# xiaojino/RUArt

Hardware: AMD Instinct MI355X
Metric: VQA samples/sec fwd+bwd (B=64, q=30, ocr=100) (higher is better)
Workload: dtype f16 MFMA + block-scaled fp8 (e4m3) MFMA correction, f32 accumulate / residual stream

## Files before the change

ruart_amd/csrc/sdnet_gemm.hip:

```cpp
#include <cstdlib>
#include "common.h"
#include "ruart_hip.h"

#define XBK 32
template <int TM> struct XT {
  static constexpr int THREADS = TM * 2;
  static constexpr int WN = TM / 64;
  static constexpr int JT = TM / 32;
  static constexpr int TRS = TM * 2 + 16;
  static constexpr int ARR = 32 * TRS;
};

typedef __attribute__((__vector_size__(4 * sizeof(short)))) short xtr16x4_t;
typedef __attribute__((address_space(3))) xtr16x4_t* xtr_ptr_t;

namespace {

__device__ __forceinline__ void split_bf16(float x, bf16_t& hi, bf16_t& lo) {
  hi = (bf16_t)x;
  lo = (bf16_t)(x - (float)hi);
}

__device__ __forceinline__ int kc_off(int r, int chunk ) {
  const int line = r >> 1;
  return line * 128 + ((((r & 1) * 4 + chunk) ^ (line & 7)) << 4);
}

template <int TM, int MODE, int VW, bool MASKED = false>
struct Stager {
  float v[16];
  unsigned mb[MASKED ? 16 / VW : 1];
  unsigned ok;

  __device__ __forceinline__ static void ldv(const float* p, float* out) {
    if (VW == 4) {
      const f32x4_t t = *reinterpret_cast<const f32x4_t*>(p);
      out[0] = t[0]; out[1] = t[1]; out[2] = t[2]; out[3] = t[3];
    } else if (VW == 2) {
      typedef float f32x2v __attribute__((ext_vector_type(2)));
      const f32x2v t = *reinterpret_cast<const f32x2v*>(p);
      out[0] = t[0]; out[1] = t[1];
    } else {
      out[0] = *p;
    }
  }
  __device__ __forceinline__ static unsigned ldm(const unsigned char* p) {
    if (VW == 4) return *reinterpret_cast<const unsigned*>(p);
    if (VW == 2) return *reinterpret_cast<const unsigned short*>(p);
    return *p;
  }

  __device__ __forceinline__ static int div_rpm(int x, float inv) { return (int)(((float)x + 0.5f) * inv); }

  __device__ __forceinline__ static void mask_rows(int (&mo)[4], int r0, int rows, int K, int tid, int rpm) {
    const float inv = 1.0f / (float)rpm;
#pragma unroll
    for (int p = 0; p < 4; ++p) mo[p] = div_rpm(min(r0 + p * (TM / 4) + (tid >> 3), rows - 1), inv) * K;
  }

  template <bool KFULL>
  __device__ __forceinline__ void load(const float* __restrict__ P, long srow, long sk, int r0, int rows, int k0, int K, int tid,
                                       const unsigned char* __restrict__ S, int rpm, const int (&mo)[4]) {
    ok = KFULL ? 0xffffu : 0u;
    if (MODE == 0) {
      const int kq = (tid & 7) * 4;
      const unsigned pitch = (unsigned)srow;
#pragma unroll
      for (int p = 0; p < 4; ++p) {
        const int r = r0 + p * (TM / 4) + (tid >> 3), k = k0 + kq;
        const unsigned ro = (unsigned)min(r, rows - 1) * pitch;
#pragma unroll
        for (int j = 0; j < 4; j += VW) {
          const int kk = k + j, kc = KFULL ? kk : min(kk, K - VW);
          ldv(P + (ro + (unsigned)kc), &v[p * 4 + j]);
          if (!KFULL && kk < K) ok |= ((1u << VW) - 1u) << (p * 4 + j);
          if (MASKED) mb[(p * 4 + j) / VW] = ldm(S + (unsigned)(mo[p] + kc));
        }
      }
    } else {
      const int m4 = (tid % (TM / 4)) * 4;
      const float inv = 1.0f / (float)rpm;
      const unsigned pitch = (unsigned)sk;
#pragma unroll
      for (int p = 0; p < 4; ++p) {
        const int k = k0 + 2 * (tid / (TM / 4)) + (p & 1) + 16 * (p >> 1), r = r0 + m4;
        const int kc = KFULL ? k : min(k, K - 1);
        const unsigned ko = (unsigned)kc * pitch;
        const unsigned so = MASKED ? (unsigned)(div_rpm(kc, inv) * rows) : 0u;
        if (!KFULL && k < K) ok |= 0xfu << (p * 4);
#pragma unroll
        for (int j = 0; j < 4; j += VW) {
          const int rrc = min(r + j, rows - VW);
          ldv(P + (ko + (unsigned)rrc), &v[p * 4 + j]);
          if (MASKED) mb[(p * 4 + j) / VW] = ldm(S + (so + (unsigned)rrc));
        }
      }
    }
  }

  template <bool KFULL>
  __device__ __forceinline__ void store(char* hi_img, char* lo_img, int tid, bool with_lo = true, float scale = 1.f) const {
#pragma unroll
    for (int p = 0; p < 4; ++p) {
      bf16x4_t h, l;
#pragma unroll
      for (int i = 0; i < 4; ++i) {
        bf16_t a, b;
        const int e = p * 4 + i;
        float x = v[e];
        if (MASKED) x = ((mb[e / VW] >> (8 * (e % VW))) & 0xffu) ? x * scale : 0.f;
        if (!KFULL) x = ((ok >> e) & 1u) ? x : 0.f;
        split_bf16(x, a, b);
        h[i] = a;
        l[i] = b;
      }
      int off;
      if (MODE == 0) {
        const int r = p * (TM / 4) + (tid >> 3), kq = tid & 7;
        off = kc_off(r, kq >> 1) + (kq & 1) * 8;
      } else {
        const int k = 2 * (tid / (TM / 4)) + (p & 1) + 16 * (p >> 1);
        off = k * XT<TM>::TRS + (tid % (TM / 4)) * 8;
      }
      *reinterpret_cast<bf16x4_t*>(hi_img + off) = h;
      if (with_lo) *reinterpret_cast<bf16x4_t*>(lo_img + off) = l;
    }
  }
};

template <int TM, int MODE>
__device__ __forceinline__ bf16x8_t frag(const char* img, int row_base, int fr, int fq) {
  if (MODE == 0) {
    return *reinterpret_cast<const bf16x8_t*>(img + kc_off(row_base + fr, fq));
  } else {
    const char* base = img + (8 * fq + (fr >> 2)) * XT<TM>::TRS + (row_base + (fr & 3) * 4) * 2;
    union { struct { xtr16x4_t a, b; } s; bf16x8_t f; } u;
    u.s.a = __builtin_amdgcn_ds_read_tr16_b64_v4i16((xtr_ptr_t)base);
    u.s.b = __builtin_amdgcn_ds_read_tr16_b64_v4i16((xtr_ptr_t)(base + 4 * XT<TM>::TRS));
    return u.f;
  }
}

template <int TM, int AMODE, int BMODE, int VWA, int VWB, int NP, int MSK = 0>
__device__ __forceinline__ void x3_tile(const float* __restrict__ A, long sam, long sak, const float* __restrict__ B, long sbk, long sbn,
                                        const float* __restrict__ bias, float* __restrict__ C, int ldc, int M, int N, int K, int splitk,
                                        float* __restrict__ ws, const unsigned char* __restrict__ a_scale, const unsigned char* __restrict__ b_scale,
                                        float keep_scale, const float* __restrict__ c_scale, int rpm, const float* __restrict__ R, int ldr,
                                        int act, int id) {
  typedef XT<TM> T;
  constexpr int ARR = T::ARR, JT = T::JT;
  extern __shared__ __attribute__((aligned(1024))) char smem[];
  const int tid = threadIdx.x, lane = tid & 63, wave = tid >> 6;
  const int wm = wave / T::WN, wn = wave % T::WN;
  const int fr = lane & 15, fq = lane >> 4;
  const int ntn = (N + TM - 1) / TM;
  const int tile = id / splitk, slice = id - tile * splitk;
  const int m0 = (tile / ntn) * TM, n0 = (tile % ntn) * TM;
  const int ksteps = (K + XBK - 1) / XBK;
  const int per = (ksteps + splitk - 1) / splitk;
  const int kbeg = slice * per, kend = min(ksteps, kbeg + per);

  f32x4_t acc[4][JT];
#pragma unroll
  for (int i = 0; i < 4; ++i)
#pragma unroll
    for (int j = 0; j < JT; ++j) acc[i][j] = (f32x4_t){0.f, 0.f, 0.f, 0.f};

  const long a_srow = sam, a_sk = sak, b_srow = sbn, b_sk = sbk;
  auto compute = [&](const char* st) {
#pragma unroll
    for (int jh = 0; jh < JT / 4; ++jh) {
      bf16x8_t ah[4], al[4];
#pragma unroll
      for (int j = 0; j < 4; ++j) {
        ah[j] = frag<TM, AMODE>(st, wm * (TM / 2) + (jh * 4 + j) * 16, fr, fq);
        if (NP == 3) al[j] = frag<TM, AMODE>(st + ARR, wm * (TM / 2) + (jh * 4 + j) * 16, fr, fq);
      }
#pragma unroll
      for (int i = 0; i < 4; ++i) {
        const bf16x8_t bh = frag<TM, BMODE>(st + 2 * ARR, wn * 64 + i * 16, fr, fq);
        bf16x8_t bl = bh;
        if (NP == 3) bl = frag<TM, BMODE>(st + 3 * ARR, wn * 64 + i * 16, fr, fq);
#pragma unroll
        for (int j = 0; j < 4; ++j) {
          f32x4_t& c = acc[i][jh * 4 + j];
          if (NP == 3) {
            c = mfma_16x16x32(bl, ah[j], c);
            c = mfma_16x16x32(bh, al[j], c);
          }
          c = mfma_16x16x32(bh, ah[j], c);
        }
      }
    }
  };
  int moa[4] = {0, 0, 0, 0}, mob[4] = {0, 0, 0, 0};
  if (MSK == 1 && AMODE == 0) Stager<TM, AMODE, VWA, true>::mask_rows(moa, m0, M, K, tid, rpm);
  if (MSK == 2 && BMODE == 0) Stager<TM, BMODE, VWB, true>::mask_rows(mob, n0, N, K, tid, rpm);
  if constexpr (TM == 128) {
    Stager<TM, AMODE, VWA, MSK == 1> sa0, sa1;
    Stager<TM, BMODE, VWB, MSK == 2> sb0, sb1;
    sa0.template load<false>(A, a_srow, a_sk, m0, M, kbeg * XBK, K, tid, a_scale, rpm, moa);
    sb0.template load<false>(B, b_srow, b_sk, n0, N, kbeg * XBK, K, tid, b_scale, rpm, mob);
    sa1.template load<false>(A, a_srow, a_sk, m0, M, (kbeg + 1) * XBK, K, tid, a_scale, rpm, moa);
    sb1.template load<false>(B, b_srow, b_sk, n0, N, (kbeg + 1) * XBK, K, tid, b_scale, rpm, mob);
    char* const st0 = smem;
    char* const st1 = smem + 4 * ARR;
    int t = kbeg;
#define X3_PAIR(KF)                                                                                       \
    {                                                                                                     \
      sa0.template store<KF>(st0, st0 + ARR, tid, NP == 3, keep_scale);                                   \
      sb0.template store<KF>(st0 + 2 * ARR, st0 + 3 * ARR, tid, NP == 3, keep_scale);                     \
      __syncthreads();                 \
      __builtin_amdgcn_sched_barrier(0);                                                                  \
      sa0.template load<KF>(A, a_srow, a_sk, m0, M, (t + 2) * XBK, K, tid, a_scale, rpm, moa);            \
      sb0.template load<KF>(B, b_srow, b_sk, n0, N, (t + 2) * XBK, K, tid, b_scale, rpm, mob);            \
      __builtin_amdgcn_sched_barrier(0);                                                                  \
      compute(st0);                                                                                       \
      __builtin_amdgcn_sched_barrier(0);                                                                  \
      sa1.template store<KF>(st1, st1 + ARR, tid, NP == 3, keep_scale);                                   \
      sb1.template store<KF>(st1 + 2 * ARR, st1 + 3 * ARR, tid, NP == 3, keep_scale);                     \
      __syncthreads();                                                                                    \
      __builtin_amdgcn_sched_barrier(0);                                                                  \
      sa1.template load<KF>(A, a_srow, a_sk, m0, M, (t + 3) * XBK, K, tid, a_scale, rpm, moa);            \
      sb1.template load<KF>(B, b_srow, b_sk, n0, N, (t + 3) * XBK, K, tid, b_scale, rpm, mob);            \
      __builtin_amdgcn_sched_barrier(0);                                                                  \
      compute(st1);                                                                                       \
      __builtin_amdgcn_sched_barrier(0);                                                                  \
    }
    const int kfull = K / XBK;
    for (; t + 1 < kend && t + 3 < kfull; t += 2) X3_PAIR(true)
    for (; t + 1 < kend; t += 2) X3_PAIR(false)
#undef X3_PAIR
    if (t < kend) {
      sa0.template store<false>(st0, st0 + ARR, tid, NP == 3, keep_scale);
      sb0.template store<false>(st0 + 2 * ARR, st0 + 3 * ARR, tid, NP == 3, keep_scale);
      __syncthreads();
      compute(st0);
    }
  } else {
    Stager<TM, AMODE, VWA, MSK == 1> sa;
    Stager<TM, BMODE, VWB, MSK == 2> sb;
    if (kbeg < kend) {
      sa.template load<false>(A, a_srow, a_sk, m0, M, kbeg * XBK, K, tid, a_scale, rpm, moa);
      sb.template load<false>(B, b_srow, b_sk, n0, N, kbeg * XBK, K, tid, b_scale, rpm, mob);
    }
    const int kfull = K / XBK;
    int t = kbeg;
    for (; t + 1 < kend && t + 1 < kfull; ++t) {
      char* st = smem + ((t - kbeg) & 1) * (4 * ARR);
      sa.template store<true>(st, st + ARR, tid, NP == 3, keep_scale);
      sb.template store<true>(st + 2 * ARR, st + 3 * ARR, tid, NP == 3, keep_scale);
      __syncthreads();
      sa.template load<true>(A, a_srow, a_sk, m0, M, (t + 1) * XBK, K, tid, a_scale, rpm, moa);
      sb.template load<true>(B, b_srow, b_sk, n0, N, (t + 1) * XBK, K, tid, b_scale, rpm, mob);
      compute(st);
    }
    for (; t < kend; ++t) {
      char* st = smem + ((t - kbeg) & 1) * (4 * ARR);
      sa.template store<false>(st, st + ARR, tid, NP == 3, keep_scale);
      sb.template store<false>(st + 2 * ARR, st + 3 * ARR, tid, NP == 3, keep_scale);
      __syncthreads();
      if (t + 1 < kend) {
        sa.template load<false>(A, a_srow, a_sk, m0, M, (t + 1) * XBK, K, tid, a_scale, rpm, moa);
        sb.template load<false>(B, b_srow, b_sk, n0, N, (t + 1) * XBK, K, tid, b_scale, rpm, mob);
      }
      compute(st);
    }
  }

  if (splitk > 1) {
    float* slab = ws + ((size_t)tile * splitk + slice) * (TM * TM);
#pragma unroll
    for (int i = 0; i < 4; ++i)
#pragma unroll
      for (int j = 0; j < JT; ++j) *reinterpret_cast<f32x4_t*>(slab + ((i * JT + j) * T::THREADS + tid) * 4) = acc[i][j];
    return;
  }
  const uintptr_t bits = reinterpret_cast<uintptr_t>(C) | (R ? reinterpret_cast<uintptr_t>(R) : 0) | (bias ? reinterpret_cast<uintptr_t>(bias) : 0) |
                         (c_scale ? reinterpret_cast<uintptr_t>(c_scale) : 0);
  const bool vec_all = (bits & 15) == 0 && (ldc & 3) == 0 && (!R || (ldr & 3) == 0) && (!c_scale || (N & 3) == 0);
#pragma unroll
  for (int i = 0; i < 4; ++i) {
    const int n = n0 + wn * 64 + i * 16 + fq * 4;
    if (vec_all && n + 3 < N) {
      f32x4_t bv = {0.f, 0.f, 0.f, 0.f};
      if (bias) bv = *reinterpret_cast<const f32x4_t*>(bias + n);
#pragma unroll
      for (int j = 0; j < JT; ++j) {
        const int m = m0 + wm * (TM / 2) + j * 16 + fr;
        if (m >= M) continue;
        f32x4_t v = acc[i][j] + bv;
        if (act == RUART_ACT_GELU) {
#pragma unroll
          for (int r = 0; r < 4; ++r) v[r] = v[r] * 0.5f * (1.0f + erff(v[r] * 0.70710678118654752440f));
        }
        if (c_scale) v *= *reinterpret_cast<const f32x4_t*>(c_scale + (size_t)(m / rpm) * N + n);
        if (R) v += *reinterpret_cast<const f32x4_t*>(R + (size_t)m * ldr + n);
        *reinterpret_cast<f32x4_t*>(C + (size_t)m * ldc + n) = v;
      }
      continue;
    }
    f32x4_t bv = {0.f, 0.f, 0.f, 0.f};
    if (bias) {
#pragma unroll
      for (int r = 0; r < 4; ++r) bv[r] = (n + r < N) ? bias[n + r] : 0.f;
    }
#pragma unroll
    for (int j = 0; j < JT; ++j) {
      const int m = m0 + wm * (TM / 2) + j * 16 + fr;
      if (m >= M || n >= N) continue;
      f32x4_t v = acc[i][j] + bv;
      if (act == RUART_ACT_GELU) {
#pragma unroll
        for (int r = 0; r < 4; ++r) v[r] = v[r] * 0.5f * (1.0f + erff(v[r] * 0.70710678118654752440f));
      }
      if (c_scale) {
        const float* sp = c_scale + (size_t)(m / rpm) * N + n;
#pragma unroll
        for (int r = 0; r < 4; ++r)
          if (n + r < N) v[r] *= sp[r];
      }
      if (R) {
        const float* rp = R + (size_t)m * ldr + n;
#pragma unroll
        for (int r = 0; r < 4; ++r)
          if (n + r < N) v[r] += rp[r];
      }
      float* dst = C + (size_t)m * ldc + n;
#pragma unroll
      for (int r = 0; r < 4; ++r)
        if (n + r < N) dst[r] = v[r];
    }
  }
}

template <int TM, int AMODE, int BMODE, int VWA, int VWB, int NP = 3, int MSK = 0>
__global__ __launch_bounds__(TM * 2, 2) void gemm_x3_kernel(const float* __restrict__ A, long sam, long sak, const float* __restrict__ B,
                                                            long sbk, long sbn, const float* __restrict__ bias, float* __restrict__ C,
                                                            int ldc, int M, int N, int K, int splitk, float* __restrict__ ws,
                                                            const unsigned char* __restrict__ a_scale,
                                                            const unsigned char* __restrict__ b_scale, float keep_scale,
                                                            const float* __restrict__ c_scale, int rpm, const float* __restrict__ R,
                                                            int ldr, int act) {
  x3_tile<TM, AMODE, BMODE, VWA, VWB, NP, MSK>(A, sam, sak, B, sbk, sbn, bias, C, ldc, M, N, K, splitk, ws, a_scale, b_scale, keep_scale, c_scale,
                                               rpm, R, ldr, act, xcd_remap(blockIdx.x, gridDim.x));
}

#define X3G_MAX 44
struct X3GProb {
  const float* A;
  const float* B;
  float* C;
  float* ws;
  int lda, ldb, ldc, M, N, K, splitk, blk0, red0, accum;
};
struct X3GArgs {
  X3GProb p[X3G_MAX];
  int n;
};
template <bool VECA, bool VECB>
__global__ __launch_bounds__(256, 2) void gemm_x3_grouped_tn_kernel(const X3GArgs g) {
  const int id = xcd_remap(blockIdx.x, gridDim.x);
  int q = 0;
  while (q + 1 < g.n && id >= g.p[q + 1].blk0) ++q;
  const X3GProb& P = g.p[q];
  const float* R = (P.accum && P.splitk == 1) ? P.C : nullptr;
  x3_tile<128, 1, 1, VECA ? 4 : 1, VECB ? 4 : 1, 3>(P.A, 1, P.lda, P.B, P.ldb, 1, nullptr, P.C, P.ldc, P.M, P.N, P.K, P.splitk, P.ws, nullptr, nullptr,
                                    1.f, nullptr, 1, R, P.ldc, RUART_ACT_NONE, id - P.blk0);
}

template <int TM>
__device__ __forceinline__ void x3_reduce_body(const float* __restrict__ ws, const float* __restrict__ bias, float* __restrict__ C, int ldc,
                                               int M, int N, int splitk, const float* __restrict__ c_scale, int rpm,
                                               const float* __restrict__ R, int ldr, int act, int blk) {
  typedef XT<TM> T;
  constexpr int JT = T::JT;
  const int tid = threadIdx.x, lane = tid & 63, wave = tid >> 6;
  const int wm = wave / T::WN, wn = wave % T::WN, fr = lane & 15, fq = lane >> 4;
  const int ntn = (N + TM - 1) / TM;
  const int tile = blk / (4 * JT), ij = blk % (4 * JT), i = ij / JT, j = ij % JT;
  const int m = (tile / ntn) * TM + wm * (TM / 2) + j * 16 + fr, n = (tile % ntn) * TM + wn * 64 + i * 16 + fq * 4;
  if (m >= M || n >= N) return;
  const float* p = ws + (size_t)tile * splitk * (TM * TM) + (ij * T::THREADS + tid) * 4;
  f32x4_t s = {0.f, 0.f, 0.f, 0.f};
  int sl = 0;
  for (; sl + 8 <= splitk; sl += 8) {
    f32x4_t a[8];
#pragma unroll
    for (int u = 0; u < 8; ++u) a[u] = *reinterpret_cast<const f32x4_t*>(p + (size_t)(sl + u) * (TM * TM));
#pragma unroll
    for (int u = 0; u < 8; ++u) s += a[u];
  }
  {
    f32x4_t a[8];
#pragma unroll
    for (int u = 0; u < 8; ++u) a[u] = *reinterpret_cast<const f32x4_t*>(p + (size_t)min(sl + u, splitk - 1) * (TM * TM));
#pragma unroll
    for (int u = 0; u < 8; ++u)
      if (sl + u < splitk) s += a[u];
  }
  const uintptr_t bits = reinterpret_cast<uintptr_t>(C) | (R ? reinterpret_cast<uintptr_t>(R) : 0) | (bias ? reinterpret_cast<uintptr_t>(bias) : 0) |
                         (c_scale ? reinterpret_cast<uintptr_t>(c_scale) : 0);
  const bool vec = n + 3 < N && (bits & 15) == 0 && (ldc & 3) == 0 && (!R || (ldr & 3) == 0) && (!c_scale || (N & 3) == 0);
  if (vec) {
    f32x4_t v = s;
    if (bias) v += *reinterpret_cast<const f32x4_t*>(bias + n);
    if (act == RUART_ACT_GELU) {
#pragma unroll
      for (int r = 0; r < 4; ++r) v[r] = v[r] * 0.5f * (1.0f + erff(v[r] * 0.70710678118654752440f));
    }
    if (c_scale) v *= *reinterpret_cast<const f32x4_t*>(c_scale + (size_t)(m / rpm) * N + n);
    if (R) v += *reinterpret_cast<const f32x4_t*>(R + (size_t)m * ldr + n);
    *reinterpret_cast<f32x4_t*>(C + (size_t)m * ldc + n) = v;
    return;
  }
#pragma unroll
  for (int r = 0; r < 4; ++r)
    if (n + r < N) {
      float v = s[r] + (bias ? bias[n + r] : 0.f);
      if (act == RUART_ACT_GELU) v = v * 0.5f * (1.0f + erff(v * 0.70710678118654752440f));
      if (c_scale) v *= c_scale[(size_t)(m / rpm) * N + n + r];
      if (R) v += R[(size_t)m * ldr + n + r];
      C[(size_t)m * ldc + n + r] = v;
    }
}

template <int TM>
__global__ __launch_bounds__(TM * 2) void x3_reduce_kernel(const float* __restrict__ ws, const float* __restrict__ bias,
                                                           float* __restrict__ C, int ldc, int M, int N, int splitk,
                                                           const float* __restrict__ c_scale, int rpm, const float* __restrict__ R,
                                                           int ldr, int act) {
  x3_reduce_body<TM>(ws, bias, C, ldc, M, N, splitk, c_scale, rpm, R, ldr, act, blockIdx.x);
}

__global__ __launch_bounds__(256) void x3_reduce_grouped_kernel(const X3GArgs g) {
  const int id = blockIdx.x;
  int q = 0;
  while (q + 1 < g.n && id >= g.p[q + 1].red0) ++q;
  const X3GProb& P = g.p[q];
  if (P.splitk <= 1) return;
  x3_reduce_body<128>(P.ws, nullptr, P.C, P.ldc, P.M, P.N, P.splitk, nullptr, 1, P.accum ? P.C : nullptr, P.ldc, RUART_ACT_NONE, id - P.red0);
}

struct Plan { int tm, tiles, splitk; };

Plan make_plan(int M, int N, int K, int amode, int bmode) {
  const int ksteps = (K + XBK - 1) / XBK;
  static const int fill = [] { const char* e = getenv("RUART_X3_FILL"); return e ? atoi(e) : 128; }();
  static const int nosplit = [] { const char* e = getenv("RUART_X3_NOSPLIT_TILES"); return e ? atoi(e) : 160; }();
  auto split_for = [&](int tiles) {
    if (tiles >= nosplit || ksteps < 16) return 1;
    int s = (fill + tiles - 1) / tiles;
    if (s > ksteps / 4) s = ksteps / 4;
    if (s > 64) s = 64;
    return s < 1 ? 1 : s;
  };
  const int t256 = ((M + 255) / 256) * ((N + 255) / 256), t128 = ((M + 127) / 128) * ((N + 127) / 128);
  Plan p;
  static const int fill256 = [] { const char* e = getenv("RUART_X3_T256_FILL"); return e ? atoi(e) : 256; }();
  static const int min256 = [] { const char* e = getenv("RUART_X3_T256_MIN"); return e ? atoi(e) : 192; }();
  int s256 = 1;
  if (t256 < 200 && ksteps >= 16) {
    s256 = (fill256 + t256 - 1) / t256;
    if (s256 > ksteps / 8) s256 = ksteps / 8;
    if (s256 < 1) s256 = 1;
  }
  const double waste = (double)t256 * 65536.0 / ((double)M * N);
  if (bmode == 0 && (long long)M * N >= 4096LL * 1024 && t256 * s256 >= min256 && waste < 1.25) {
    (void)amode;
    p.tm = 256; p.tiles = t256; p.splitk = s256;
  } else {
    p.tm = 128; p.tiles = t128; p.splitk = split_for(t128);
  }
  return p;
}

template <int TM, int AM, int BM_, int VA, int VB, int NP = 3, int MSK = 0>
void launch_x3(const float* A, long sam, long sak, const float* B, long sbk, long sbn, const float* bias, float* C, int ldc, int M,
               int N, int K, const Plan& p, float* ws, const unsigned char* a_scale, const unsigned char* b_scale, float keep_scale,
               const float* c_scale, int rpm,
               const float* R, int ldr, int act, hipStream_t s) {
  auto kern = gemm_x3_kernel<TM, AM, BM_, VA, VB, NP, MSK>;
  constexpr int lds = 2 * 4 * XT<TM>::ARR;
  static bool done = (hipFuncSetAttribute((const void*)kern, hipFuncAttributeMaxDynamicSharedMemorySize, lds), true);
  (void)done;
  hipLaunchKernelGGL(kern, dim3(p.tiles * p.splitk), dim3(XT<TM>::THREADS), lds, s, A, sam, sak, B, sbk, sbn, bias, C, ldc, M, N, K,
                     p.splitk, ws, a_scale, b_scale, keep_scale, c_scale, rpm, R, ldr, act);
  if (p.splitk > 1)
    hipLaunchKernelGGL(x3_reduce_kernel<TM>, dim3(p.tiles * 4 * XT<TM>::JT), dim3(XT<TM>::THREADS), 0, s, ws, bias, C, ldc, M, N, p.splitk,
                       c_scale, rpm, R, ldr, act);
}

}

extern "C" int ruart_gemm_x3_plan(int M, int N, int K, int a_k_contiguous, int b_k_contiguous, int* splitk, size_t* ws_bytes) {
  RUART_ENTRY();
  if (M <= 0 || N <= 0 || K <= 0) return (int)hipErrorInvalidValue;
  const Plan p = make_plan(M, N, K, a_k_contiguous ? 0 : 1, b_k_contiguous ? 0 : 1);
  if (splitk) *splitk = p.splitk;
  if (ws_bytes) *ws_bytes = p.splitk > 1 ? (size_t)p.tiles * p.splitk * p.tm * p.tm * sizeof(float) : 0;
  return 0;
}

namespace {
template <int NP>
int gemm_xn(const float* A, long long sam, long long sak, const float* B, long long sbk, long long sbn,
            const float* bias, const float* residual, int ldr, int act, float* C, int ldc, int M, int N, int K,
            float* ws, size_t ws_bytes, const unsigned char* a_scale, const unsigned char* b_scale, float keep_scale,
            const float* c_scale, int rows_per_scale_row, void* stream) {
  if (!A || !B || !C || M <= 0 || N <= 0 || K <= 0 || ldc < N) return (int)hipErrorInvalidValue;
  if ((residual && ldr < N) || (act != RUART_ACT_NONE && act != RUART_ACT_GELU)) return (int)hipErrorInvalidValue;
  const float* R = residual;
  const int rpm = rows_per_scale_row > 0 ? rows_per_scale_row : 1;
  if ((a_scale && sak != 1) || (b_scale && sbn != 1)) return (int)hipErrorInvalidValue;
  const int amode = (sak == 1) ? 0 : (sam == 1 ? 1 : -1);
  const int bmode = (sbk == 1) ? 0 : (sbn == 1 ? 1 : -1);
  if (amode < 0 || bmode < 0) return (int)hipErrorInvalidValue;
  {
    const long long ea = amode == 0 ? (long long)(M - 1) * sam + K : (long long)(K - 1) * sak + M;
    const long long eb = bmode == 0 ? (long long)(N - 1) * sbn + K : (long long)(K - 1) * sbk + N;
    if (ea >= (1LL << 30) || eb >= (1LL << 30) || sam < 0 || sak < 0 || sbk < 0 || sbn < 0) return (int)hipErrorInvalidValue;
  }
  Plan p = make_plan(M, N, K, amode, bmode);
  if (p.splitk > 1 && (!ws || ws_bytes < (size_t)p.tiles * p.splitk * p.tm * p.tm * sizeof(float))) p.splitk = 1;
  auto width = [](const float* base, long pitch, int extent, const unsigned char* mask) {
    const uintptr_t bits = reinterpret_cast<uintptr_t>(base), mbits = mask ? reinterpret_cast<uintptr_t>(mask) : 0;
    if ((bits & 15) == 0 && (mbits & 3) == 0 && (pitch & 3) == 0 && (extent & 3) == 0) return 4;
    if ((bits & 7) == 0 && (mbits & 1) == 0 && (pitch & 1) == 0 && (extent & 1) == 0) return 2;
    return 1;
  };
  const int vwa = width(A, amode == 0 ? sam : sak, amode == 0 ? K : M, a_scale);
  const int vwb = width(B, bmode == 0 ? sbn : sbk, bmode == 0 ? K : N, b_scale);
  if (p.tm == 256 && (vwa == 1 || vwb == 1)) {
    p.tm = 128;
    p.tiles = ((M + 127) / 128) * ((N + 127) / 128);
    p.splitk = 1;
  }
  hipStream_t s = (hipStream_t)stream;
#define X3L(TM, AM, BM_, VA, VB) \
  launch_x3<TM, AM, BM_, VA, VB, NP>(A, sam, sak, B, sbk, sbn, bias, C, ldc, M, N, K, p, ws, a_scale, b_scale, keep_scale, c_scale, rpm, R, ldr, act, s)
#define X3W(TM, AM, BM_)                                         \
  do {                                                           \
    if (vwa == 4 && vwb == 4) X3L(TM, AM, BM_, 4, 4);            \
    else if (vwa == 4 && vwb == 2) X3L(TM, AM, BM_, 4, 2);       \
    else if (vwa == 2 && vwb == 4) X3L(TM, AM, BM_, 2, 4);       \
    else if (vwa == 2 && vwb == 2) X3L(TM, AM, BM_, 2, 2);       \
    else if (TM == 256) return (int)hipErrorInvalidValue;        \
    else X3S(AM, BM_);                                           \
  } while (0)
#define X3S(AM, BM_)                                             \
  do {                                                           \
    if (vwa == 4) X3L(128, AM, BM_, 4, 1);                       \
    else if (vwa == 2) X3L(128, AM, BM_, 2, 1);                  \
    else if (vwb == 4) X3L(128, AM, BM_, 1, 4);                  \
    else if (vwb == 2) X3L(128, AM, BM_, 1, 2);                  \
    else X3L(128, AM, BM_, 1, 1);                                \
  } while (0)
  if (a_scale || b_scale) {
    if (a_scale && b_scale) return (int)hipErrorInvalidValue;
    const int vw = vwa < vwb ? vwa : vwb;
#define X3M(TM, AM, BM_, VW_, MSK_) \
  launch_x3<TM, AM, BM_, VW_, VW_, NP, MSK_>(A, sam, sak, B, sbk, sbn, bias, C, ldc, M, N, K, p, ws, a_scale, b_scale, keep_scale, c_scale, rpm, R, ldr, act, s)
    if (a_scale && amode == 0 && bmode == 0) {
      if (p.tm == 256 && vw >= 2) {
        if (vw == 4) X3M(256, 0, 0, 4, 1); else X3M(256, 0, 0, 2, 1);
      } else {
        if (p.tm == 256) { p.tm = 128; p.tiles = ((M + 127) / 128) * ((N + 127) / 128); p.splitk = 1; }
        if (vw == 4) X3M(128, 0, 0, 4, 1); else if (vw == 2) X3M(128, 0, 0, 2, 1); else X3M(128, 0, 0, 1, 1);
      }
    } else {
      if (p.tm == 256) { p.tm = 128; p.tiles = ((M + 127) / 128) * ((N + 127) / 128); p.splitk = 1; }
      if (b_scale && amode == 1 && bmode == 1) {
        if (vw == 4) X3M(128, 1, 1, 4, 2); else if (vw == 2) X3M(128, 1, 1, 2, 2); else X3M(128, 1, 1, 1, 2);
      } else if (a_scale && amode == 0 && bmode == 1) X3M(128, 0, 1, 1, 1);
      else if (b_scale && amode == 0 && bmode == 1) X3M(128, 0, 1, 1, 2);
      else return (int)hipErrorInvalidValue;
    }
#undef X3M
  } else if (p.tm == 256) {
    if (bmode != 0) return (int)hipErrorInvalidValue;
    if (amode == 0) X3W(256, 0, 0); else X3W(256, 1, 0);
  } else if (amode == 0 && bmode == 0) X3W(128, 0, 0);
  else if (amode == 0 && bmode == 1) X3W(128, 0, 1);
  else if (amode == 1 && bmode == 0) X3W(128, 1, 0);
  else X3W(128, 1, 1);
#undef X3S
#undef X3W
#undef X3L
  RUART_CHECK_LAUNCH();
  return 0;
}
}

extern "C" int ruart_gemm_x3(const float* A, long long sam, long long sak, const float* B, long long sbk, long long sbn,
                             const float* bias, const float* residual, int ldr, int act, float* C, int ldc, int M, int N, int K,
                             float* ws, size_t ws_bytes, const unsigned char* a_keep, const unsigned char* b_keep, float keep_scale,
                             const float* c_scale, int rows_per_scale_row, void* stream) {
  RUART_ENTRY();
  return gemm_xn<3>(A, sam, sak, B, sbk, sbn, bias, residual, ldr, act, C, ldc, M, N, K, ws, ws_bytes, a_keep, b_keep, keep_scale, c_scale,
                    rows_per_scale_row, stream);
}

extern "C" int ruart_gemm_x1(const float* A, long long sam, long long sak, const float* B, long long sbk, long long sbn,
                             const float* bias, const float* residual, int ldr, int act, float* C, int ldc, int M, int N, int K,
                             float* ws, size_t ws_bytes, const unsigned char* a_keep, const unsigned char* b_keep, float keep_scale,
                             const float* c_scale, int rows_per_scale_row, void* stream) {
  RUART_ENTRY();
  return gemm_xn<1>(A, sam, sak, B, sbk, sbn, bias, residual, ldr, act, C, ldc, M, N, K, ws, ws_bytes, a_keep, b_keep, keep_scale, c_scale,
                    rows_per_scale_row, stream);
}

extern "C" int ruart_gemm_bf16_tn(const float* A, long long sak_rows, const float* B, long long sbk_rows, float* C, int ldc, int M, int N,
                                  int K, float* ws, size_t ws_bytes, void* stream) {
  RUART_ENTRY();
  return gemm_xn<1>(A, 1, sak_rows, B, sbk_rows, 1, nullptr, nullptr, 0, RUART_ACT_NONE, C, ldc, M, N, K, ws, ws_bytes, nullptr, nullptr,
                    1.f, nullptr, 1, stream);
}

extern "C" size_t ruart_gemm_x3_tn_grouped_ws(const ruart_x3_tn_problem* probs, int n) {
  size_t total = 0;
  for (int i = 0; i < n; ++i) {
    const Plan p = make_plan(probs[i].M, probs[i].N, probs[i].K, 1, 1);
    if (p.splitk > 1) total += (size_t)p.tiles * p.splitk * 128 * 128 * sizeof(float);
  }
  return total;
}

extern "C" int ruart_gemm_x3_tn_grouped(const ruart_x3_tn_problem* probs, int n, float* ws, size_t ws_bytes, void* stream) {
  RUART_ENTRY();
  if (n <= 0 || !probs) return (int)hipErrorInvalidValue;
  if (ruart_gemm_x3_tn_grouped_ws(probs, n) > ws_bytes) return (int)hipErrorInvalidValue;
  hipStream_t s = (hipStream_t)stream;
  size_t ws_off = 0;
  for (int cls = 0; cls < 4; ++cls) {
    const bool va = cls & 1, vb = cls & 2;
    X3GArgs g;
    g.n = 0;
    int blk = 0, red = 0;
    auto flush = [&]() -> int {
      if (g.n == 0) return 0;
      constexpr int lds = 2 * 4 * XT<128>::ARR;
#define X3G_LAUNCH(VA, VB)                                                                                                  \
  do {                                                                                                                       \
    auto kern = gemm_x3_grouped_tn_kernel<VA, VB>;                                                                           \
    static bool done = (hipFuncSetAttribute((const void*)kern, hipFuncAttributeMaxDynamicSharedMemorySize, lds), true);    \
    (void)done;                                                                                                              \
    hipLaunchKernelGGL(kern, dim3(blk), dim3(256), lds, s, g);                                                               \
  } while (0)
      if (va && vb) X3G_LAUNCH(true, true);
      else if (va) X3G_LAUNCH(true, false);
      else if (vb) X3G_LAUNCH(false, true);
      else X3G_LAUNCH(false, false);
#undef X3G_LAUNCH
      hipError_t e = hipGetLastError();
      if (e != hipSuccess) return (int)e;
      if (red > 0) {
        hipLaunchKernelGGL(x3_reduce_grouped_kernel, dim3(red), dim3(256), 0, s, g);
        e = hipGetLastError();
        if (e != hipSuccess) return (int)e;
      }
      g.n = 0;
      blk = red = 0;
      return 0;
    };
    for (int i = 0; i < n; ++i) {
      const ruart_x3_tn_problem& q = probs[i];
      if (!q.A || !q.B || !q.C || q.M <= 0 || q.N <= 0 || q.K <= 0 || q.lda < q.M || q.ldb < q.N || q.ldc < q.N ||
          (long long)q.K * q.lda >= (1LL << 30) || (long long)q.K * q.ldb >= (1LL << 30))
        return (int)hipErrorInvalidValue;
      const bool qa = ((reinterpret_cast<uintptr_t>(q.A) & 15) == 0) && ((q.lda & 3) == 0) && ((q.M & 3) == 0);
      const bool qb = ((reinterpret_cast<uintptr_t>(q.B) & 15) == 0) && ((q.ldb & 3) == 0) && ((q.N & 3) == 0);
      if (qa != va || qb != vb) continue;
      const Plan pl = make_plan(q.M, q.N, q.K, 1, 1);
      X3GProb& P = g.p[g.n];
      P.A = q.A; P.B = q.B; P.C = q.C;
      P.lda = q.lda; P.ldb = q.ldb; P.ldc = q.ldc;
      P.M = q.M; P.N = q.N; P.K = q.K;
      P.splitk = pl.splitk;
      P.accum = q.accumulate ? 1 : 0;
      P.blk0 = blk;
      P.red0 = red;
      P.ws = nullptr;
      if (pl.splitk > 1) {
        P.ws = ws + ws_off / sizeof(float);
        ws_off += (size_t)pl.tiles * pl.splitk * 128 * 128 * sizeof(float);
        red += pl.tiles * 4 * XT<128>::JT;
      }
      blk += pl.tiles * pl.splitk;
      if (++g.n == X3G_MAX) {
        const int rc = flush();
        if (rc) return rc;
      }
    }
    const int rc = flush();
    if (rc) return rc;
  }
  return 0;
}
```

Measured before the change: 2895.

## Use unaligned 4-wide loads with edge shifting instead of alignment-gated width dispatch

Replaces the alignment-based vector-width selection (4/2/1) in the fp32-input GEMM staging with a single rule: use 4-wide loads whenever the extent is at least 4, using unaligned vector types. Edge tiles clamp the load start and then shift the loaded lanes in registers to realign them, so misaligned or odd-sized operands no longer fall back to scalar or 2-wide loads or drop from 256 to 128 tiles. The epilogue and split-K reduce also drop the alignment check and use unaligned 4-wide stores. This adds select logic at edge tiles and relies on unaligned global accesses being cheap.

```diff
diff --git a/ruart_amd/csrc/sdnet_gemm.hip b/ruart_amd/csrc/sdnet_gemm.hip
--- a/ruart_amd/csrc/sdnet_gemm.hip
+++ b/ruart_amd/csrc/sdnet_gemm.hip
@@ -26,27 +26,29 @@
   return line * 128 + ((((r & 1) * 4 + chunk) ^ (line & 7)) << 4);
 }
 
+typedef float f32x4u_t __attribute__((ext_vector_type(4), aligned(4)));
+
 template <int TM, int MODE, int VW, bool MASKED = false>
 struct Stager {
+  static_assert(VW == 4 || VW == 1, "one vector width; the element form serves extents below 4");
   float v[16];
   unsigned mb[MASKED ? 16 / VW : 1];
   unsigned ok;
 
   __device__ __forceinline__ static void ldv(const float* p, float* out) {
     if (VW == 4) {
-      const f32x4_t t = *reinterpret_cast<const f32x4_t*>(p);
+      const f32x4u_t t = *reinterpret_cast<const f32x4u_t*>(p);
       out[0] = t[0]; out[1] = t[1]; out[2] = t[2]; out[3] = t[3];
-    } else if (VW == 2) {
-      typedef float f32x2v __attribute__((ext_vector_type(2)));
-      const f32x2v t = *reinterpret_cast<const f32x2v*>(p);
-      out[0] = t[0]; out[1] = t[1];
     } else {
       out[0] = *p;
     }
   }
   __device__ __forceinline__ static unsigned ldm(const unsigned char* p) {
-    if (VW == 4) return *reinterpret_cast<const unsigned*>(p);
-    if (VW == 2) return *reinterpret_cast<const unsigned short*>(p);
+    if (VW == 4) {
+      unsigned u;
+      __builtin_memcpy(&u, p, 4);
+      return u;
+    }
     return *p;
   }
 
@@ -61,20 +63,32 @@
   template <bool KFULL>
   __device__ __forceinline__ void load(const float* __restrict__ P, long srow, long sk, int r0, int rows, int k0, int K, int tid,
                                        const unsigned char* __restrict__ S, int rpm, const int (&mo)[4]) {
-    ok = KFULL ? 0xffffu : 0u;
+    ok = KFULL ? (VW == 4 && MODE == 0 ? 0u : 0xffffu) : 0u;
     if (MODE == 0) {
       const int kq = (tid & 7) * 4;
       const unsigned pitch = (unsigned)srow;
-#pragma unroll
-      for (int p = 0; p < 4; ++p) {
-        const int r = r0 + p * (TM / 4) + (tid >> 3), k = k0 + kq;
-        const unsigned ro = (unsigned)min(r, rows - 1) * pitch;
-#pragma unroll
-        for (int j = 0; j < 4; j += VW) {
-          const int kk = k + j, kc = KFULL ? kk : min(kk, K - VW);
-          ldv(P + (ro + (unsigned)kc), &v[p * 4 + j]);
-          if (!KFULL && kk < K) ok |= ((1u << VW) - 1u) << (p * 4 + j);
-          if (MASKED) mb[(p * 4 + j) / VW] = ldm(S + (unsigned)(mo[p] + kc));
+      if (VW == 4) {
+        const int k = k0 + kq, kc = KFULL ? k : min(k, K - 4);
+        if (!KFULL) ok = (unsigned)min(k - kc, 4);
+#pragma unroll
+        for (int p = 0; p < 4; ++p) {
+          const int r = r0 + p * (TM / 4) + (tid >> 3);
+          const unsigned ro = (unsigned)min(r, rows - 1) * pitch;
+          ldv(P + (ro + (unsigned)kc), &v[p * 4]);
+          if (MASKED) mb[p] = ldm(S + (unsigned)(mo[p] + kc));
+        }
+      } else {
+#pragma unroll
+        for (int p = 0; p < 4; ++p) {
+          const int r = r0 + p * (TM / 4) + (tid >> 3), k = k0 + kq;
+          const unsigned ro = (unsigned)min(r, rows - 1) * pitch;
+#pragma unroll
+          for (int j = 0; j < 4; ++j) {
+            const int kk = k + j, kc = KFULL ? kk : min(kk, K - 1);
+            ldv(P + (ro + (unsigned)kc), &v[p * 4 + j]);
+            if (!KFULL && kk < K) ok |= 1u << (p * 4 + j);
+            if (MASKED) mb[p * 4 + j] = ldm(S + (unsigned)(mo[p] + kc));
+          }
         }
       }
     } else {
@@ -99,7 +113,31 @@
   }
 
   template <bool KFULL>
-  __device__ __forceinline__ void store(char* hi_img, char* lo_img, int tid, bool with_lo = true, float scale = 1.f) const {
+  __device__ __forceinline__ void store(char* hi_img, char* lo_img, int tid, int r0, int rows, bool with_lo = true, float scale = 1.f) {
+    if (VW == 4 && MODE == 0 && !KFULL) {
+      const unsigned sh = ok;
+#pragma unroll
+      for (int p = 0; p < 4; ++p) {
+        const float t0 = v[p * 4], t1 = v[p * 4 + 1], t2 = v[p * 4 + 2], t3 = v[p * 4 + 3];
+        v[p * 4] = sh == 0 ? t0 : sh == 1 ? t1 : sh == 2 ? t2 : sh == 3 ? t3 : 0.f;
+        v[p * 4 + 1] = sh == 0 ? t1 : sh == 1 ? t2 : sh == 2 ? t3 : 0.f;
+        v[p * 4 + 2] = sh == 0 ? t2 : sh == 1 ? t3 : 0.f;
+        v[p * 4 + 3] = sh == 0 ? t3 : 0.f;
+        if (MASKED) mb[p] >>= 8 * min(sh, 3u);
+      }
+    }
+    if (VW == 4 && MODE == 1 && r0 + TM > rows && (rows & 3) != 0) {
+      const int r = r0 + (tid % (TM / 4)) * 4;
+      const int sh = r - min(r, rows - 4);
+#pragma unroll
+      for (int p = 0; p < 4; ++p) {
+        const float t0 = v[p * 4], t1 = v[p * 4 + 1], t2 = v[p * 4 + 2], t3 = v[p * 4 + 3];
+        v[p * 4] = sh == 0 ? t0 : sh == 1 ? t1 : sh == 2 ? t2 : t3;
+        v[p * 4 + 1] = sh == 0 ? t1 : sh == 1 ? t2 : sh == 2 ? t3 : t1;
+        v[p * 4 + 2] = sh == 1 ? t3 : t2;
+        if (MASKED) mb[p] >>= 8 * min(sh, 3);
+      }
+    }
 #pragma unroll
     for (int p = 0; p < 4; ++p) {
       bf16x4_t h, l;
@@ -109,7 +147,7 @@
         const int e = p * 4 + i;
         float x = v[e];
         if (MASKED) x = ((mb[e / VW] >> (8 * (e % VW))) & 0xffu) ? x * scale : 0.f;
-        if (!KFULL) x = ((ok >> e) & 1u) ? x : 0.f;
+        if (!KFULL && !(VW == 4 && MODE == 0)) x = ((ok >> e) & 1u) ? x : 0.f;
         split_bf16(x, a, b);
         h[i] = a;
         l[i] = b;
@@ -208,8 +246,8 @@
     int t = kbeg;
 #define X3_PAIR(KF)                                                                                       \
     {                                                                                                     \
-      sa0.template store<KF>(st0, st0 + ARR, tid, NP == 3, keep_scale);                                   \
-      sb0.template store<KF>(st0 + 2 * ARR, st0 + 3 * ARR, tid, NP == 3, keep_scale);                     \
+      sa0.template store<KF>(st0, st0 + ARR, tid, m0, M, NP == 3, keep_scale);                                   \
+      sb0.template store<KF>(st0 + 2 * ARR, st0 + 3 * ARR, tid, n0, N, NP == 3, keep_scale);                     \
       __syncthreads();                 \
       __builtin_amdgcn_sched_barrier(0);                                                                  \
       sa0.template load<KF>(A, a_srow, a_sk, m0, M, (t + 2) * XBK, K, tid, a_scale, rpm, moa);            \
@@ -217,8 +255,8 @@
       __builtin_amdgcn_sched_barrier(0);                                                                  \
       compute(st0);                                                                                       \
       __builtin_amdgcn_sched_barrier(0);                                                                  \
-      sa1.template store<KF>(st1, st1 + ARR, tid, NP == 3, keep_scale);                                   \
-      sb1.template store<KF>(st1 + 2 * ARR, st1 + 3 * ARR, tid, NP == 3, keep_scale);                     \
+      sa1.template store<KF>(st1, st1 + ARR, tid, m0, M, NP == 3, keep_scale);                                   \
+      sb1.template store<KF>(st1 + 2 * ARR, st1 + 3 * ARR, tid, n0, N, NP == 3, keep_scale);                     \
       __syncthreads();                                                                                    \
       __builtin_amdgcn_sched_barrier(0);                                                                  \
       sa1.template load<KF>(A, a_srow, a_sk, m0, M, (t + 3) * XBK, K, tid, a_scale, rpm, moa);            \
@@ -232,8 +270,8 @@
     for (; t + 1 < kend; t += 2) X3_PAIR(false)
 #undef X3_PAIR
     if (t < kend) {
-      sa0.template store<false>(st0, st0 + ARR, tid, NP == 3, keep_scale);
-      sb0.template store<false>(st0 + 2 * ARR, st0 + 3 * ARR, tid, NP == 3, keep_scale);
+      sa0.template store<false>(st0, st0 + ARR, tid, m0, M, NP == 3, keep_scale);
+      sb0.template store<false>(st0 + 2 * ARR, st0 + 3 * ARR, tid, n0, N, NP == 3, keep_scale);
       __syncthreads();
       compute(st0);
     }
@@ -248,8 +286,8 @@
     int t = kbeg;
     for (; t + 1 < kend && t + 1 < kfull; ++t) {
       char* st = smem + ((t - kbeg) & 1) * (4 * ARR);
-      sa.template store<true>(st, st + ARR, tid, NP == 3, keep_scale);
-      sb.template store<true>(st + 2 * ARR, st + 3 * ARR, tid, NP == 3, keep_scale);
+      sa.template store<true>(st, st + ARR, tid, m0, M, NP == 3, keep_scale);
+      sb.template store<true>(st + 2 * ARR, st + 3 * ARR, tid, n0, N, NP == 3, keep_scale);
       __syncthreads();
       sa.template load<true>(A, a_srow, a_sk, m0, M, (t + 1) * XBK, K, tid, a_scale, rpm, moa);
       sb.template load<true>(B, b_srow, b_sk, n0, N, (t + 1) * XBK, K, tid, b_scale, rpm, mob);
@@ -257,8 +295,8 @@
     }
     for (; t < kend; ++t) {
       char* st = smem + ((t - kbeg) & 1) * (4 * ARR);
-      sa.template store<false>(st, st + ARR, tid, NP == 3, keep_scale);
-      sb.template store<false>(st + 2 * ARR, st + 3 * ARR, tid, NP == 3, keep_scale);
+      sa.template store<false>(st, st + ARR, tid, m0, M, NP == 3, keep_scale);
+      sb.template store<false>(st + 2 * ARR, st + 3 * ARR, tid, n0, N, NP == 3, keep_scale);
       __syncthreads();
       if (t + 1 < kend) {
         sa.template load<false>(A, a_srow, a_sk, m0, M, (t + 1) * XBK, K, tid, a_scale, rpm, moa);
@@ -276,15 +314,12 @@
       for (int j = 0; j < JT; ++j) *reinterpret_cast<f32x4_t*>(slab + ((i * JT + j) * T::THREADS + tid) * 4) = acc[i][j];
     return;
   }
-  const uintptr_t bits = reinterpret_cast<uintptr_t>(C) | (R ? reinterpret_cast<uintptr_t>(R) : 0) | (bias ? reinterpret_cast<uintptr_t>(bias) : 0) |
-                         (c_scale ? reinterpret_cast<uintptr_t>(c_scale) : 0);
-  const bool vec_all = (bits & 15) == 0 && (ldc & 3) == 0 && (!R || (ldr & 3) == 0) && (!c_scale || (N & 3) == 0);
 #pragma unroll
   for (int i = 0; i < 4; ++i) {
     const int n = n0 + wn * 64 + i * 16 + fq * 4;
-    if (vec_all && n + 3 < N) {
+    if (n + 3 < N) {
       f32x4_t bv = {0.f, 0.f, 0.f, 0.f};
-      if (bias) bv = *reinterpret_cast<const f32x4_t*>(bias + n);
+      if (bias) bv = *reinterpret_cast<const f32x4u_t*>(bias + n);
 #pragma unroll
       for (int j = 0; j < JT; ++j) {
         const int m = m0 + wm * (TM / 2) + j * 16 + fr;
@@ -294,9 +329,9 @@
 #pragma unroll
           for (int r = 0; r < 4; ++r) v[r] = v[r] * 0.5f * (1.0f + erff(v[r] * 0.70710678118654752440f));
         }
-        if (c_scale) v *= *reinterpret_cast<const f32x4_t*>(c_scale + (size_t)(m / rpm) * N + n);
-        if (R) v += *reinterpret_cast<const f32x4_t*>(R + (size_t)m * ldr + n);
-        *reinterpret_cast<f32x4_t*>(C + (size_t)m * ldc + n) = v;
+        if (c_scale) v *= *reinterpret_cast<const f32x4u_t*>(c_scale + (size_t)(m / rpm) * N + n);
+        if (R) v += *reinterpret_cast<const f32x4u_t*>(R + (size_t)m * ldr + n);
+        *reinterpret_cast<f32x4u_t*>(C + (size_t)m * ldc + n) = v;
       }
       continue;
     }
@@ -358,14 +393,14 @@
   X3GProb p[X3G_MAX];
   int n;
 };
-template <bool VECA, bool VECB>
+template <int VWA, int VWB>
 __global__ __launch_bounds__(256, 2) void gemm_x3_grouped_tn_kernel(const X3GArgs g) {
   const int id = xcd_remap(blockIdx.x, gridDim.x);
   int q = 0;
   while (q + 1 < g.n && id >= g.p[q + 1].blk0) ++q;
   const X3GProb& P = g.p[q];
   const float* R = (P.accum && P.splitk == 1) ? P.C : nullptr;
-  x3_tile<128, 1, 1, VECA ? 4 : 1, VECB ? 4 : 1, 3>(P.A, 1, P.lda, P.B, P.ldb, 1, nullptr, P.C, P.ldc, P.M, P.N, P.K, P.splitk, P.ws, nullptr, nullptr,
+  x3_tile<128, 1, 1, VWA, VWB, 3>(P.A, 1, P.lda, P.B, P.ldb, 1, nullptr, P.C, P.ldc, P.M, P.N, P.K, P.splitk, P.ws, nullptr, nullptr,
                                     1.f, nullptr, 1, R, P.ldc, RUART_ACT_NONE, id - P.blk0);
 }
 
@@ -399,19 +434,16 @@
     for (int u = 0; u < 8; ++u)
       if (sl + u < splitk) s += a[u];
   }
-  const uintptr_t bits = reinterpret_cast<uintptr_t>(C) | (R ? reinterpret_cast<uintptr_t>(R) : 0) | (bias ? reinterpret_cast<uintptr_t>(bias) : 0) |
-                         (c_scale ? reinterpret_cast<uintptr_t>(c_scale) : 0);
-  const bool vec = n + 3 < N && (bits & 15) == 0 && (ldc & 3) == 0 && (!R || (ldr & 3) == 0) && (!c_scale || (N & 3) == 0);
-  if (vec) {
+  if (n + 3 < N) {
     f32x4_t v = s;
-    if (bias) v += *reinterpret_cast<const f32x4_t*>(bias + n);
+    if (bias) v += *reinterpret_cast<const f32x4u_t*>(bias + n);
     if (act == RUART_ACT_GELU) {
 #pragma unroll
       for (int r = 0; r < 4; ++r) v[r] = v[r] * 0.5f * (1.0f + erff(v[r] * 0.70710678118654752440f));
     }
-    if (c_scale) v *= *reinterpret_cast<const f32x4_t*>(c_scale + (size_t)(m / rpm) * N + n);
-    if (R) v += *reinterpret_cast<const f32x4_t*>(R + (size_t)m * ldr + n);
-    *reinterpret_cast<f32x4_t*>(C + (size_t)m * ldc + n) = v;
+    if (c_scale) v *= *reinterpret_cast<const f32x4u_t*>(c_scale + (size_t)(m / rpm) * N + n);
+    if (R) v += *reinterpret_cast<const f32x4u_t*>(R + (size_t)m * ldr + n);
+    *reinterpret_cast<f32x4u_t*>(C + (size_t)m * ldc + n) = v;
     return;
   }
 #pragma unroll
@@ -466,7 +498,7 @@
     if (s256 < 1) s256 = 1;
   }
   const double waste = (double)t256 * 65536.0 / ((double)M * N);
-  if (bmode == 0 && (long long)M * N >= 4096LL * 1024 && t256 * s256 >= min256 && waste < 1.25) {
+  if (bmode == 0 && (long long)M * N >= 4096LL * 1024 && t256 * s256 >= min256 && waste < 1.25 && M >= 4 && K >= 4) {
     (void)amode;
     p.tm = 256; p.tiles = t256; p.splitk = s256;
   } else {
@@ -523,68 +555,37 @@
   }
   Plan p = make_plan(M, N, K, amode, bmode);
   if (p.splitk > 1 && (!ws || ws_bytes < (size_t)p.tiles * p.splitk * p.tm * p.tm * sizeof(float))) p.splitk = 1;
-  auto width = [](const float* base, long pitch, int extent, const unsigned char* mask) {
-    const uintptr_t bits = reinterpret_cast<uintptr_t>(base), mbits = mask ? reinterpret_cast<uintptr_t>(mask) : 0;
-    if ((bits & 15) == 0 && (mbits & 3) == 0 && (pitch & 3) == 0 && (extent & 3) == 0) return 4;
-    if ((bits & 7) == 0 && (mbits & 1) == 0 && (pitch & 1) == 0 && (extent & 1) == 0) return 2;
-    return 1;
-  };
-  const int vwa = width(A, amode == 0 ? sam : sak, amode == 0 ? K : M, a_scale);
-  const int vwb = width(B, bmode == 0 ? sbn : sbk, bmode == 0 ? K : N, b_scale);
-  if (p.tm == 256 && (vwa == 1 || vwb == 1)) {
-    p.tm = 128;
-    p.tiles = ((M + 127) / 128) * ((N + 127) / 128);
-    p.splitk = 1;
-  }
+  const int vwa = (amode == 0 ? K : M) >= 4 ? 4 : 1;
+  const int vwb = (bmode == 0 ? K : N) >= 4 ? 4 : 1;
   hipStream_t s = (hipStream_t)stream;
-#define X3L(TM, AM, BM_, VA, VB) \
-  launch_x3<TM, AM, BM_, VA, VB, NP>(A, sam, sak, B, sbk, sbn, bias, C, ldc, M, N, K, p, ws, a_scale, b_scale, keep_scale, c_scale, rpm, R, ldr, act, s)
-#define X3W(TM, AM, BM_)                                         \
+#define X3L(TM, AM, BM_, VA, VB, MSK_) \
+  launch_x3<TM, AM, BM_, VA, VB, NP, MSK_>(A, sam, sak, B, sbk, sbn, bias, C, ldc, M, N, K, p, ws, a_scale, b_scale, keep_scale, c_scale, rpm, R, ldr, act, s)
+#define X3W(AM, BM_, MSK_)                                       \
   do {                                                           \
-    if (vwa == 4 && vwb == 4) X3L(TM, AM, BM_, 4, 4);            \
-    else if (vwa == 4 && vwb == 2) X3L(TM, AM, BM_, 4, 2);       \
-    else if (vwa == 2 && vwb == 4) X3L(TM, AM, BM_, 2, 4);       \
-    else if (vwa == 2 && vwb == 2) X3L(TM, AM, BM_, 2, 2);       \
-    else if (TM == 256) return (int)hipErrorInvalidValue;        \
-    else X3S(AM, BM_);                                           \
+    if (vwa == 4 && vwb == 4) X3L(128, AM, BM_, 4, 4, MSK_);     \
+    else if (vwa == 4) X3L(128, AM, BM_, 4, 1, MSK_);            \
+    else if (vwb == 4) X3L(128, AM, BM_, 1, 4, MSK_);            \
+    else X3L(128, AM, BM_, 1, 1, MSK_);                          \
   } while (0)
-#define X3S(AM, BM_)                                             \
-  do {                                                           \
-    if (vwa == 4) X3L(128, AM, BM_, 4, 1);                       \
-    else if (vwa == 2) X3L(128, AM, BM_, 2, 1);                  \
-    else if (vwb == 4) X3L(128, AM, BM_, 1, 4);                  \
-    else if (vwb == 2) X3L(128, AM, BM_, 1, 2);                  \
-    else X3L(128, AM, BM_, 1, 1);                                \
-  } while (0)
+  if (p.tm == 256 && (vwa != 4 || vwb != 4 || bmode != 0)) return (int)hipErrorInvalidValue;
   if (a_scale || b_scale) {
     if (a_scale && b_scale) return (int)hipErrorInvalidValue;
-    const int vw = vwa < vwb ? vwa : vwb;
-#define X3M(TM, AM, BM_, VW_, MSK_) \
-  launch_x3<TM, AM, BM_, VW_, VW_, NP, MSK_>(A, sam, sak, B, sbk, sbn, bias, C, ldc, M, N, K, p, ws, a_scale, b_scale, keep_scale, c_scale, rpm, R, ldr, act, s)
     if (a_scale && amode == 0 && bmode == 0) {
-      if (p.tm == 256 && vw >= 2) {
-        if (vw == 4) X3M(256, 0, 0, 4, 1); else X3M(256, 0, 0, 2, 1);
-      } else {
-        if (p.tm == 256) { p.tm = 128; p.tiles = ((M + 127) / 128) * ((N + 127) / 128); p.splitk = 1; }
-        if (vw == 4) X3M(128, 0, 0, 4, 1); else if (vw == 2) X3M(128, 0, 0, 2, 1); else X3M(128, 0, 0, 1, 1);
-      }
+      if (p.tm == 256) X3L(256, 0, 0, 4, 4, 1);
+      else X3W(0, 0, 1);
     } else {
       if (p.tm == 256) { p.tm = 128; p.tiles = ((M + 127) / 128) * ((N + 127) / 128); p.splitk = 1; }
-      if (b_scale && amode == 1 && bmode == 1) {
-        if (vw == 4) X3M(128, 1, 1, 4, 2); else if (vw == 2) X3M(128, 1, 1, 2, 2); else X3M(128, 1, 1, 1, 2);
-      } else if (a_scale && amode == 0 && bmode == 1) X3M(128, 0, 1, 1, 1);
-      else if (b_scale && amode == 0 && bmode == 1) X3M(128, 0, 1, 1, 2);
+      if (b_scale && amode == 1 && bmode == 1) X3W(1, 1, 2);
+      else if (a_scale && amode == 0 && bmode == 1) X3W(0, 1, 1);
+      else if (b_scale && amode == 0 && bmode == 1) X3W(0, 1, 2);
       else return (int)hipErrorInvalidValue;
     }
-#undef X3M
   } else if (p.tm == 256) {
-    if (bmode != 0) return (int)hipErrorInvalidValue;
-    if (amode == 0) X3W(256, 0, 0); else X3W(256, 1, 0);
-  } else if (amode == 0 && bmode == 0) X3W(128, 0, 0);
-  else if (amode == 0 && bmode == 1) X3W(128, 0, 1);
-  else if (amode == 1 && bmode == 0) X3W(128, 1, 0);
-  else X3W(128, 1, 1);
-#undef X3S
+    if (amode == 0) X3L(256, 0, 0, 4, 4, 0); else X3L(256, 1, 0, 4, 4, 0);
+  } else if (amode == 0 && bmode == 0) X3W(0, 0, 0);
+  else if (amode == 0 && bmode == 1) X3W(0, 1, 0);
+  else if (amode == 1 && bmode == 0) X3W(1, 0, 0);
+  else X3W(1, 1, 0);
 #undef X3W
 #undef X3L
   RUART_CHECK_LAUNCH();
@@ -647,10 +648,10 @@
     (void)done;                                                                                                              \
     hipLaunchKernelGGL(kern, dim3(blk), dim3(256), lds, s, g);                                                               \
   } while (0)
-      if (va && vb) X3G_LAUNCH(true, true);
-      else if (va) X3G_LAUNCH(true, false);
-      else if (vb) X3G_LAUNCH(false, true);
-      else X3G_LAUNCH(false, false);
+      if (va && vb) X3G_LAUNCH(4, 4);
+      else if (va) X3G_LAUNCH(4, 1);
+      else if (vb) X3G_LAUNCH(1, 4);
+      else X3G_LAUNCH(1, 1);
 #undef X3G_LAUNCH
       hipError_t e = hipGetLastError();
       if (e != hipSuccess) return (int)e;
@@ -668,8 +669,7 @@
       if (!q.A || !q.B || !q.C || q.M <= 0 || q.N <= 0 || q.K <= 0 || q.lda < q.M || q.ldb < q.N || q.ldc < q.N ||
           (long long)q.K * q.lda >= (1LL << 30) || (long long)q.K * q.ldb >= (1LL << 30))
         return (int)hipErrorInvalidValue;
-      const bool qa = ((reinterpret_cast<uintptr_t>(q.A) & 15) == 0) && ((q.lda & 3) == 0) && ((q.M & 3) == 0);
-      const bool qb = ((reinterpret_cast<uintptr_t>(q.B) & 15) == 0) && ((q.ldb & 3) == 0) && ((q.N & 3) == 0);
+      const bool qa = q.M >= 4, qb = q.N >= 4;
       if (qa != va || qb != vb) continue;
       const Plan pl = make_plan(q.M, q.N, q.K, 1, 1);
       X3GProb& P = g.p[g.n];
```

New measurement: 2894. Within noise of the previous version (-0.0%).
